# PRBonn/OverlapNet

Measured on NVIDIA H100. Metric: scan-pairs/sec (overlap+yaw) at 64x900, higher is better.
Workload: dtype f16

## Files before the change

### overlapnet_b200/csrc/network_tc.cu

```cuda
#include "common.cuh"
#include "hopper.cuh"

#include <cuda_fp16.h>
#include <stddef.h>
#include <stdlib.h>

namespace ovn {

using namespace hopper;

constexpr int WF = 360;
constexpr int CF = 128;
constexpr int S15 = 15;
constexpr int NB = 24;
constexpr int PAIR_ROWS = NB * NB;
constexpr int K4_PITCH = CF;

struct TcState {
  Buffer<__half> w1p;
  Buffer<__half> w2p;
  Buffer<__half> w3p;
  Buffer<float> b2eff;
  Buffer<__half> wres[kMaxLegLayers];
  Buffer<__half> actp[2];
// ... 463 lines not shown
              wgmma_m64n128k16_ss(acc[sub], desc_kmajor(a_base + sub * (C2_TILE / 2) + kk * 32, 16, 1024, kSwizzle128B), bd);
          }
        wgmma_commit();
        wgmma_wait<1>();
        if (di > 0) S.ring.release(gi - 1);
      }
      wgmma_wait<0>();
      if (failed) goto done;
      S.ring.release(gi - 1);
#pragma unroll
      for (int sub = 0; sub < 2; ++sub)
#pragma unroll
        for (int h = 0; h < 2; ++h) {
          const int64_t m = tile * TC_ROWS + wg * 128 + sub * 64 + wi * 16 + g + 8 * h;
          if (m >= M) continue;
#pragma unroll
          for (int j = 0; j < 16; ++j) {
            const int n = j * 8 + 2 * t;
            const float a = fmaxf(acc[sub][4 * j + 2 * h] + __ldg(bias2 + n), 0.f) - __ldg(mu_x3 + n);
            const float b = fmaxf(acc[sub][4 * j + 2 * h + 1] + __ldg(bias2 + n + 1), 0.f) - __ldg(mu_x3 + n + 1);
            *reinterpret_cast<uint32_t*>(x3 + ((size_t)j * out_pitch + m) * 8 + 2 * t) = pack_h2(a, b);
          }
        }
    }
  }
done:
  return;
}

constexpr int C3_AROWS = TC_ROWS + 2 * NB + 2;
constexpr uint32_t C3_PLANE = C3_AROWS * 16;
constexpr uint32_t C3_SLAB = 4 * 128 * 16;
constexpr int C3_GROUP = 2;
constexpr int C3_NSTAGES = 36 / C3_GROUP;
constexpr int C3_RING = 4;

struct C3Smem {
  __half A[2][16 * C3_PLANE / 2];
  __half B[C3_RING][C3_GROUP * C3_SLAB / 2];
  MbarRing<C3_RING> w3;
  MbarRing<2> x3;
};
static_assert(sizeof(C3Smem) <= 232448, "k_conv3_wgmma shared memory");
static_assert(offsetof(C3Smem, B) % 16 == 0 && C3_PLANE % 16 == 0, "bulk-copy alignment");

__global__ void __launch_bounds__(TC_THREADS, 1)
k_conv3_wgmma(const __half* __restrict__ X3, int64_t a_pitch, const __half* __restrict__ W3p, const float* __restrict__ bias,
              int64_t M, const float* __restrict__ wd, float* __restrict__ partial, int* __restrict__ err) {
  extern __shared__ __align__(128) uint8_t smem_raw[];
  C3Smem& S = *reinterpret_cast<C3Smem*>(smem_raw);
  const int tid = threadIdx.x, warp = tid >> 5, lane = tid & 31;
  const Share tiles = work_share(2 * ((M + TC_ROWS - 1) / TC_ROWS), blockIdx.x, gridDim.x);
  if (tid == 0) {
    S.w3.init(TC_WG * 4);
    S.x3.init(TC_WG * 4);
    mbar_fence_init();
  }
  __syncthreads();

  if (warp == TC_WG * 4) {
    if (lane == 0) {
      const uint32_t nt = (uint32_t)(tiles.end - tiles.begin);
      uint32_t ai = 0, gi = 0;
      for (uint32_t ti = 0; ti < nt; ++ti) {
        const int nh = (int)((tiles.begin + ti) & 1);
        for (int st = 0; st < C3_NSTAGES; ++st, ++gi) {
          while (ai < nt && ai <= ti + 1) {
            if (ai > ti) {
              if (!S.x3.try_acquire(ai, 16 * C3_PLANE)) break;
            } else {
              PIPE_WAIT(S.x3.acquire(ai, 16 * C3_PLANE), kErrConv3X3Producer);
            }
            const int64_t r0 = ((tiles.begin + ai) >> 1) * TC_ROWS;
            for (int pl = 0; pl < 16; ++pl)
              bulk_g2s(S.A[S.x3.slot(ai)] + pl * (C3_PLANE / 2), X3 + ((size_t)pl * a_pitch + r0) * 8, C3_PLANE, S.x3.bar(ai));
            ++ai;
          }
          PIPE_WAIT(S.w3.acquire(gi, C3_GROUP * C3_SLAB), kErrConv3W3Producer);
          bulk_g2s(S.B[S.w3.slot(gi)], W3p + ((size_t)nh * 36 + st * C3_GROUP) * (C3_SLAB / 2), C3_GROUP * C3_SLAB,
                   S.w3.bar(gi));
        }
      }
    }
  } else {
    const int wg = warp >> 2, wi = warp & 3, g = lane >> 2, t = lane & 3;
    const uint32_t b_base = smem_u32(S.B[0]);
    uint32_t gi = 0;
    bool failed = false;
    for (int64_t tile = tiles.begin; tile < tiles.end; ++tile) {
      const uint32_t ti = (uint32_t)(tile - tiles.begin);
      const int nh = (int)(tile & 1);
      const int64_t r0 = (tile >> 1) * TC_ROWS;
      PIPE_WAIT(S.x3.wait(ti), kErrConv3X3Consumer);
      const uint32_t a_rows = smem_u32(S.A[S.x3.slot(ti)]) + wg * 128 * 16;
      float acc[2][64];
#pragma unroll
      for (int sub = 0; sub < 2; ++sub)
#pragma unroll
        for (int e = 0; e < 64; ++e) acc[sub][e] = 0.f;
#pragma unroll 1
      for (int st = 0; st < C3_NSTAGES; ++st, ++gi) {
        const uint32_t s = S.w3.slot(gi);
        INFLIGHT_WAIT(S.w3.wait(gi), kErrConv3W3Consumer);
        wgmma_fence();
#pragma unroll
        for (int sl = 0; sl < C3_GROUP; ++sl) {
          const int slab = st * C3_GROUP + sl, tap = slab >> 2, c32 = slab & 3;
          const uint32_t a_tap = a_rows + ((tap / 3) * NB + tap % 3) * 16;
          const uint32_t slab_addr = b_base + s * (C3_GROUP * C3_SLAB) + sl * C3_SLAB;
#pragma unroll
          for (int kk = 0; kk < 2; ++kk) {
            const int c16 = c32 * 2 + kk;
            const uint64_t bd = desc_kmajor(slab_addr + kk * 4096, 2048, 128, kNoSwizzle);
#pragma unroll
            for (int sub = 0; sub < 2; ++sub)
              wgmma_m64n128k16_ss(acc[sub], desc_kmajor(a_tap + 2 * c16 * C3_PLANE + sub * 64 * 16, C3_PLANE, 128, kNoSwizzle), bd);
          }
        }
        wgmma_commit();
        wgmma_wait<1>();
        if (st > 0) S.w3.release(gi - 1);
      }
      wgmma_wait<0>();
      if (failed) goto done;
      S.w3.release(gi - 1);
      S.x3.release(ti);
#pragma unroll
      for (int sub = 0; sub < 2; ++sub)
#pragma unroll
        for (int h = 0; h < 2; ++h) {
          const int64_t r = r0 + wg * 128 + sub * 64 + wi * 16 + g + 8 * h;
          const int rem = (int)(r % PAIR_ROWS);
          const int yy = rem / NB, xx = rem - yy * NB;
          const bool valid = (r < M) && (yy < NB - 2) && (xx < NB - 2);
          const float* wrow = wd + (size_t)(valid ? (xx * (NB - 2) + yy) : 0) * 256 + nh * 128;
          float sum = 0.f;
#pragma unroll
          for (int j = 0; j < 16; ++j) {
            const int n = j * 8 + 2 * t;
            sum = fmaf(fmaxf(acc[sub][4 * j + 2 * h] + __ldg(bias + nh * 128 + n), 0.f), __ldg(wrow + n), sum);
            sum = fmaf(fmaxf(acc[sub][4 * j + 2 * h + 1] + __ldg(bias + nh * 128 + n + 1), 0.f), __ldg(wrow + n + 1), sum);
          }
          sum += __shfl_xor_sync(0xffffffffu, sum, 1);
          sum += __shfl_xor_sync(0xffffffffu, sum, 2);
          if (t == 0 && r < M) partial[r * 2 + nh] = valid ? sum : 0.f;
        }
    }
  }
done:
  return;
}

constexpr int C6_PARTS = C6_LT * C6_RT;
constexpr int C6_WG = 2;
constexpr int C6_THREADS = C6_WG * 128 + 32;
constexpr int C6_RING = 3;
constexpr int C6_GPITCH = 132;

struct C6Smem {
  __half R[C6_R_BYTES / 2];
  __half L[C6_RING][C6_L_BYTES / 2];
  float G[C6_WG][C6_LROWS * C6_GPITCH];
  MbarRing<C6_RING> left;
  MbarRing<1> right;
};
static_assert(sizeof(C6Smem) <= 232448, "k_corr_wgmma shared memory");
static_assert(offsetof(C6Smem, L) % 16 == 0, "bulk-copy alignment");

__global__ void __launch_bounds__(C6_THREADS, 1)
k_corr_wgmma(const __half* __restrict__ Lc, const int32_t* __restrict__ l_idx, const __half* __restrict__ Rc,
             int r_per_pair, int n_pairs, float* __restrict__ corr_part, int* __restrict__ err) {
  extern __shared__ __align__(128) uint8_t smem_raw[];
  C6Smem& S = *reinterpret_cast<C6Smem*>(smem_raw);
  const int tid = threadIdx.x, warp = tid >> 5, lane = tid & 31;
  const int q = blockIdx.x % C6_RT;
  const Share share = work_share((int64_t)n_pairs * C6_LT, blockIdx.x / C6_RT, gridDim.x / C6_RT);
  const int u_begin = (int)share.begin, u_end = (int)share.end;
  if (tid == 0) {
    S.left.init(4);
    S.right.init(C6_WG * 4);
    mbar_fence_init();
  }
  __syncthreads();

  if (warp == C6_WG * 4) {
    if (lane == 0) {
      uint32_t ri = 0, ui = 0;
      int key = -1;
      for (int u = u_begin; u < u_end; ++u, ++ui) {
        const int p = u / C6_LT, a = u - p * C6_LT;
        if ((r_per_pair ? p : 0) != key) {
          key = r_per_pair ? p : 0;
          PIPE_WAIT(S.right.acquire(ri, C6_R_BYTES), kErrCorrRightProducer);
          bulk_g2s(S.R, Rc + ((size_t)key * C6_RT + q) * (C6_R_BYTES / 2), C6_R_BYTES, S.right.bar(ri));
          ++ri;
        }
        PIPE_WAIT(S.left.acquire(ui, C6_L_BYTES), kErrCorrLeftProducer);
        bulk_g2s(S.L[S.left.slot(ui)], Lc + ((size_t)(l_idx ? l_idx[p] : p) * C6_LT + a) * (C6_L_BYTES / 2), C6_L_BYTES,
                 S.left.bar(ui));
      }
    }
  } else {
    const int wg = warp >> 2, wi = warp & 3, g = lane >> 2, t = lane & 3, tw = tid & 127;
    float* Gw = S.G[wg];
    const uint32_t r_base = smem_u32(S.R);
    uint32_t ri = 0, ui = 0;
    int key = -1;
    bool failed = false;
    for (int u = u_begin; u < u_end; ++u, ++ui) {
      const int p = u / C6_LT, a = u - p * C6_LT;
      if ((r_per_pair ? p : 0) != key) {
        if (key >= 0) S.right.release(ri - 1);
        key = r_per_pair ? p : 0;
        INFLIGHT_WAIT(S.right.wait(ri), kErrCorrRightConsumer);
        ++ri;
      }
      if ((int)(ui & 1) != wg) continue;
      const uint32_t s = S.left.slot(ui);
      INFLIGHT_WAIT(S.left.wait(ui), kErrCorrLeftConsumer);
      const uint32_t l_base = smem_u32(S.L[s]);
      float acc[64];
#pragma unroll
      for (int e = 0; e < 64; ++e) acc[e] = 0.f;
      wgmma_fence();
#pragma unroll
      for (int c16 = 0; c16 < 8; ++c16) {
        const uint64_t ah = desc_kmajor(l_base + c16 * 2 * C6_LROWS * 16, C6_LROWS * 16, 128, kNoSwizzle);
        const uint64_t al = desc_kmajor(l_base + C6_L_BYTES / 2 + c16 * 2 * C6_LROWS * 16, C6_LROWS * 16, 128, kNoSwizzle);
        const uint64_t bh = desc_kmajor(r_base + c16 * 2 * C6_RROWS * 16, C6_RROWS * 16, 128, kNoSwizzle);
        const uint64_t bl = desc_kmajor(r_base + C6_R_BYTES / 2 + c16 * 2 * C6_RROWS * 16, C6_RROWS * 16, 128, kNoSwizzle);
        wgmma_m64n128k16_ss(acc, ah, bh);
        wgmma_m64n128k16_ss(acc, al, bh);
        wgmma_m64n128k16_ss(acc, ah, bl);
      }
      wgmma_commit();
      wgmma_wait<0>();
      S.left.release(ui);
      named_bar_sync(1 + wg, 128);
#pragma unroll
      for (int j = 0; j < 16; ++j) {
        float* r0 = Gw + (wi * 16 + g) * C6_GPITCH + j * 8 + 2 * t;
        *reinterpret_cast<float2*>(r0) = make_float2(acc[4 * j], acc[4 * j + 1]);
        *reinterpret_cast<float2*>(r0 + 8 * C6_GPITCH) = make_float2(acc[4 * j + 2], acc[4 * j + 3]);
      }
      named_bar_sync(1 + wg, 128);
      const int i_lim = min(C6_LROWS, WF - a * C6_LROWS), j_lim = min(C6_RROWS, WF - q * C6_RROWS);
      float* out = corr_part + ((size_t)p * C6_PARTS + a * C6_RT + q) * WF;
      for (int d = tw; d < WF; d += 128) {
        const int dd = d - (C6_RROWS - 1);
        float sum = 0.f;
        if (d < C6_LROWS + C6_RROWS - 1) {
#pragma unroll 8
          for (int ii = 0; ii < C6_LROWS; ++ii) {
            const int jj = ii - dd;
            if (ii < i_lim && jj >= 0 && jj < j_lim) sum += Gw[ii * C6_GPITCH + jj];
          }
        }
        int k = (a * C6_LROWS - q * C6_RROWS + dd - WF / 2) % WF;
        if (k < 0) k += WF;
        out[k] = sum;
      }
    }
  }
done:
  return;
}

template <int EPI>
__global__ void __launch_bounds__(MMA_THREADS)
k_leg_mma(LegArgs g) {
  const int warp = threadIdx.x >> 5, lane = threadIdx.x & 31, gq = lane >> 2, t = lane & 3;
  const int64_t px0 = (int64_t)blockIdx.y * MMA_ROWS + warp * 16;
  if (px0 >= g.M) return;
  const int nz = (g.n_valid + 63) / 64;
  const int y = blockIdx.x, z = blockIdx.z % nz, slice = blockIdx.z / nz;
  const int64_t in_base = (int64_t)(y / g.runs_per_img) * g.in_img_planes + (int64_t)(y % g.runs_per_img) * g.in_run_planes;
  const int64_t pa = px0 + gq < g.M ? px0 + gq : g.M - 1, pb = px0 + gq + 8 < g.M ? px0 + gq + 8 : g.M - 1;
  const int n_slabs = g.kh * g.kw * 3;
  const size_t plane = (size_t)g.a_pitch * 8;
  const int per_tap = g.c8in / 2, n_it = g.kh * g.kw * per_tap;
  const int it0 = n_it * slice / g.n_split, it1 = n_it * (slice + 1) / g.n_split;
  float acc[8][4] = {};
#pragma unroll 1
  for (int it = it0; it < it1;) {
    const int tap = it / per_tap, dh = tap / g.kw, dw = tap - dh * g.kw;
    const int c8_end = (tap + 1) * per_tap < it1 ? g.c8in : (it1 - tap * per_tap) * 2;
    {
      const __half* Ah = g.A + (size_t)(in_base + (int64_t)dh * 2 * g.c8in) * plane + (size_t)dw * 8 + 2 * t;
      const __half* Al = Ah + (size_t)g.c8in * plane;
      const __half* Bh = g.Bp + ((size_t)(z * n_slabs + (dh * g.kw + dw) * 3) * g.c8in * 64 + gq) * 8 + 2 * t;
      const __half* Bl = Bh + (size_t)2 * g.c8in * 64 * 8;
#pragma unroll 1
      for (int c8 = (it - tap * per_tap) * 2; c8 < c8_end; c8 += 2) {
        const size_t o0 = (size_t)c8 * plane, o1 = o0 + plane;
        const uint32_t h0 = ld_h2(Ah + o0 + pa * 8), h1 = ld_h2(Ah + o0 + pb * 8), h2 = ld_h2(Ah + o1 + pa * 8), h3 = ld_h2(Ah + o1 + pb * 8);
        const uint32_t l0 = ld_h2(Al + o0 + pa * 8), l1 = ld_h2(Al + o0 + pb * 8), l2 = ld_h2(Al + o1 + pa * 8), l3 = ld_h2(Al + o1 + pb * 8);
        const size_t bo = (size_t)c8 * 64 * 8;
#pragma unroll
        for (int j = 0; j < 8; ++j) {
          const uint32_t wh0 = ld_h2(Bh + bo + j * 64), wh1 = ld_h2(Bh + bo + 64 * 8 + j * 64);
          const uint32_t wl0 = ld_h2(Bl + bo + j * 64), wl1 = ld_h2(Bl + bo + 64 * 8 + j * 64);
          mma16816(acc[j], h0, h1, h2, h3, wh0, wh1);
          mma16816(acc[j], l0, l1, l2, l3, wh0, wh1);
          mma16816(acc[j], h0, h1, h2, h3, wl0, wl1);
        }
      }
    }
    it = tap * per_tap + c8_end / 2;
  }
#pragma unroll
  for (int h = 0; h < 2; ++h) {
    const int64_t px = px0 + gq + 8 * h;
    if (px >= g.M) continue;
#pragma unroll
    for (int j = 0; j < 8; ++j) {
      const int n = z * 64 + j * 8 + 2 * t;
      if (n >= g.n_valid) continue;
      if (EPI == 5) {
        *reinterpret_cast<float2*>(g.part + (((size_t)slice * gridDim.x + y) * g.M + px) * g.n_valid + n) =
            make_float2(acc[j][2 * h], acc[j][2 * h + 1]);
        continue;
      }
      const float pre_a = acc[j][2 * h] + __ldg(g.bias + n), pre_b = acc[j][2 * h + 1] + __ldg(g.bias + n + 1);
      const float a = fmaxf(pre_a, 0.f), b = fmaxf(pre_b, 0.f);
      if (EPI == 4) {
        if (leg_act_unstorable(pre_a) || leg_act_unstorable(pre_b)) atomicCAS(g.err, 0, kErrNonFiniteOperand);
        const __half2 hi = __floats2half2_rn(a, b);
        const float2 hf = __half22float2(hi);
        const int64_t pl = (int64_t)y * g.out_run_planes + (n >> 3);
        *reinterpret_cast<__half2*>(g.out_planes + ((size_t)pl * g.out_pitch + px) * 8 + (n & 7)) = hi;
        *reinterpret_cast<uint32_t*>(g.out_planes + ((size_t)(pl + g.out_run_planes / 2) * g.out_pitch + px) * 8 + (n & 7)) =
            pack_h2(a - hf.x, b - hf.y);
      } else {
        *reinterpret_cast<float2*>(g.out_f32 + ((size_t)y * g.M + px) * g.n_valid + n) = make_float2(a, b);
      }
    }
  }
}

template <int EPI>
__global__ void __launch_bounds__(256)
k_leg_splitk_reduce(LegArgs g, int rows) {
  const int c8n = g.n_valid / 8;
  const int64_t i = (int64_t)blockIdx.x * blockDim.x + threadIdx.x;
  if (i >= (int64_t)rows * g.M * c8n) return;
  const int c8 = (int)(i % c8n);
  const int64_t px = (i / c8n) % g.M, y = i / c8n / g.M;
  const int64_t slice_stride = (int64_t)rows * g.M * g.n_valid;
  const float* src = g.part + (y * g.M + px) * g.n_valid + c8 * 8;
  float v[8] = {};
  for (int sl = 0; sl < g.n_split; ++sl) {
    const float4 a = __ldg(reinterpret_cast<const float4*>(src + sl * slice_stride));
    const float4 b = __ldg(reinterpret_cast<const float4*>(src + sl * slice_stride + 4));
    v[0] += a.x; v[1] += a.y; v[2] += a.z; v[3] += a.w; v[4] += b.x; v[5] += b.y; v[6] += b.z; v[7] += b.w;
  }
  bool bad = false;
#pragma unroll
  for (int e = 0; e < 8; ++e) {
    v[e] += __ldg(g.bias + c8 * 8 + e);
    bad |= leg_act_unstorable(v[e]);
    v[e] = fmaxf(v[e], 0.f);
  }
  if (EPI == 4) {
    if (bad) atomicCAS(g.err, 0, kErrNonFiniteOperand);
    __half hi[8], lo[8];
#pragma unroll
    for (int e = 0; e < 8; ++e) {
      hi[e] = __float2half_rn(v[e]);
      lo[e] = __float2half_rn(v[e] - __half2float(hi[e]));
    }
    const int64_t pl = y * g.out_run_planes + c8;
    *reinterpret_cast<uint4*>(g.out_planes + ((size_t)pl * g.out_pitch + px) * 8) = *reinterpret_cast<const uint4*>(hi);
    *reinterpret_cast<uint4*>(g.out_planes + ((size_t)(pl + g.out_run_planes / 2) * g.out_pitch + px) * 8) =
        *reinterpret_cast<const uint4*>(lo);
  } else {
    float* dst = g.out_f32 + (y * g.M + px) * g.n_valid + c8 * 8;
    *reinterpret_cast<float4*>(dst) = make_float4(v[0], v[1], v[2], v[3]);
    *reinterpret_cast<float4*>(dst + 4) = make_float4(v[4], v[5], v[6], v[7]);
  }
}

__global__ void __launch_bounds__(384)
k_corr_finalize(const float* __restrict__ part, float* __restrict__ corr_out, int32_t* __restrict__ yaw,
                const int* __restrict__ err) {
  __shared__ float s_corr[WF];
  const int p = blockIdx.x;
  for (int k = threadIdx.x; k < WF; k += blockDim.x) {
    float c = 0.f;
    for (int b = 0; b < C6_PARTS; ++b) c += part[((size_t)p * C6_PARTS + b) * WF + k];
    s_corr[k] = c;
    if (corr_out) corr_out[(size_t)p * WF + k] = c;
  }
  __syncthreads();
  if (threadIdx.x == 0) {
    int best = 0;
    float bv = s_corr[0];
    for (int k = 1; k < WF; ++k)
      if (s_corr[k] > bv) { bv = s_corr[k]; best = k; }
    yaw[p] = (*err != 0) ? INT32_MIN : 180 - best;
  }
}

__global__ void __launch_bounds__(1024)
k_o1_channel_mean(const __half* __restrict__ o1, int64_t M, float* __restrict__ mu) {
  __shared__ float part[16][64];
  const int o = threadIdx.x & 63, g = threadIdx.x >> 6;
  float acc = 0.f;
  for (int64_t m = g; m < M; m += 16)
    for (int di = 0; di < S15; ++di) acc += __half2float(o1[o1_chunk_offset(m, di, o >> 3) + (o & 7)]);
  part[g][o] = acc;
  __syncthreads();
  if (g == 0) {
    float t = 0.f;
    for (int k = 0; k < 16; ++k) t += part[k][o];
    mu[o] = __half2float(__float2half_rn(t / (float)(M * S15)));
  }
}

__global__ void __launch_bounds__(1024)
k_x3_channel_mean(const __half* __restrict__ x3, int64_t pitch, int64_t M, float* __restrict__ mu) {
  __shared__ float part[8][128];
  const int n = threadIdx.x & 127, g = threadIdx.x >> 7;
  float acc = 0.f;
  for (int64_t m = g; m < M; m += 8) acc += __half2float(x3[((size_t)(n >> 3) * pitch + m) * 8 + (n & 7)]);
  part[g][n] = acc;
  __syncthreads();
  if (g == 0) {
    float t = 0.f;
    for (int k = 0; k < 8; ++k) t += part[k][n];
    mu[n] = t / (float)M;
  }
}

__global__ void __launch_bounds__(128)
k_fold_bias2(const float* __restrict__ b2base, const float* __restrict__ mu_o1, const float* __restrict__ W2,
             float* __restrict__ b2eff) {
  const int n = threadIdx.x;
  float acc = b2base[n];
  for (int di = 0; di < S15; ++di)
    for (int o = 0; o < 64; ++o) acc = fmaf(mu_o1[o], W2[((size_t)di * 64 + o) * 128 + n], acc);
  b2eff[n] = acc;
}

__global__ void __launch_bounds__(256)
k_fold_bias3(const float* __restrict__ b3, const float* __restrict__ mu_x3, const float* __restrict__ W3,
             float* __restrict__ b3eff) {
  const int m = threadIdx.x;
  float acc = b3[m];
  for (int tap = 0; tap < 9; ++tap)
    for (int n = 0; n < 128; ++n)
      acc = fmaf(mu_x3[n], W3[((size_t)tap * 128 + n) * 256 + m], acc);
  b3eff[m] = acc;
}

__global__ void __launch_bounds__(256)
k_dense_finalize(const float* __restrict__ partial, const float* __restrict__ bd, int rows_per_pair,
                 float* __restrict__ overlap, const int* __restrict__ err) {
  __shared__ float red[256];
  const int p = blockIdx.x;
  const float* x = partial + (size_t)p * rows_per_pair * 2;
  float acc = 0.f;
  for (int i = threadIdx.x; i < rows_per_pair * 2; i += 256) acc += x[i];
  red[threadIdx.x] = acc;
  __syncthreads();
  for (int o = 128; o > 0; o >>= 1) {
    if (threadIdx.x < o) red[threadIdx.x] += red[threadIdx.x + o];
    __syncthreads();
  }
  if (threadIdx.x == 0) overlap[p] = (*err != 0) ? __int_as_float(0x7fc00000) : 1.0f / (1.0f + expf(-(red[0] + bd[0])));
}

constexpr size_t L1_DIRECT_SMEM = 48 * 1024;
constexpr size_t L1_SMALL_SMEM = 200 * 1024;

template <bool CIN4>
__global__ void __launch_bounds__(512, CIN4 ? 0 : 2)
k_leg_layer1_direct(const float* __restrict__ x, const float* __restrict__ w, const float* __restrict__ bias,
                    int n, int H_in, int W_in, int cin, int kh, int kw, int sh, int sw, int H_out, int W_out,
                    int relu, __half* __restrict__ out, int* __restrict__ err) {
  constexpr int CO = 16;
  extern __shared__ __align__(16) float w_s[];
  const int pairs = (W_out + 1) / 2;
  int64_t idx = (int64_t)blockIdx.x * blockDim.x + threadIdx.x;
  const bool active = idx < (int64_t)n * H_out * pairs;
  if (!active) idx = 0;
  const int xo = 2 * (int)(idx % pairs);
  const int64_t r = idx / pairs;
  const int y = (int)(r % H_out);
  const int64_t img = r / H_out;
  const bool has1 = xo + 1 < W_out;
  float acc0[CO], acc1[CO];
#pragma unroll
  for (int e = 0; e < CO; ++e) acc0[e] = acc1[e] = bias[e];
  const float* base0 = x + ((img * H_in + (int64_t)y * sh) * W_in + (int64_t)xo * sw) * cin;
  const float* base1 = has1 ? base0 + (int64_t)sw * cin : base0;
  for (int dh = 0; dh < kh; ++dh) {
    __syncthreads();
    for (int i = threadIdx.x; i < kw * cin * CO; i += blockDim.x) w_s[i] = w[(size_t)dh * kw * cin * CO + i];
    __syncthreads();
    for (int dw = 0; dw < kw; ++dw) {
      const int64_t off = ((int64_t)dh * W_in + dw) * cin;
      const float* pw = w_s + (size_t)(dw * cin) * CO;
      if (CIN4) {
        const float4 a = __ldg(reinterpret_cast<const float4*>(base0 + off));
        const float4 b = __ldg(reinterpret_cast<const float4*>(base1 + off));
        const float va[4] = {a.x, a.y, a.z, a.w}, vb[4] = {b.x, b.y, b.z, b.w};
#pragma unroll
        for (int c = 0; c < 4; ++c) {
#pragma unroll
          for (int q4 = 0; q4 < 4; ++q4) {
            const float4 wv = *reinterpret_cast<const float4*>(pw + c * CO + q4 * 4);
            acc0[q4 * 4 + 0] = fmaf(va[c], wv.x, acc0[q4 * 4 + 0]); acc1[q4 * 4 + 0] = fmaf(vb[c], wv.x, acc1[q4 * 4 + 0]);
            acc0[q4 * 4 + 1] = fmaf(va[c], wv.y, acc0[q4 * 4 + 1]); acc1[q4 * 4 + 1] = fmaf(vb[c], wv.y, acc1[q4 * 4 + 1]);
            acc0[q4 * 4 + 2] = fmaf(va[c], wv.z, acc0[q4 * 4 + 2]); acc1[q4 * 4 + 2] = fmaf(vb[c], wv.z, acc1[q4 * 4 + 2]);
            acc0[q4 * 4 + 3] = fmaf(va[c], wv.w, acc0[q4 * 4 + 3]); acc1[q4 * 4 + 3] = fmaf(vb[c], wv.w, acc1[q4 * 4 + 3]);
          }
        }
      } else {
        for (int c = 0; c < cin; ++c) {
          const float va = __ldg(base0 + off + c), vb = __ldg(base1 + off + c);
#pragma unroll
          for (int q4 = 0; q4 < 4; ++q4) {
            const float4 wv = *reinterpret_cast<const float4*>(pw + c * CO + q4 * 4);
            acc0[q4 * 4 + 0] = fmaf(va, wv.x, acc0[q4 * 4 + 0]); acc1[q4 * 4 + 0] = fmaf(vb, wv.x, acc1[q4 * 4 + 0]);
            acc0[q4 * 4 + 1] = fmaf(va, wv.y, acc0[q4 * 4 + 1]); acc1[q4 * 4 + 1] = fmaf(vb, wv.y, acc1[q4 * 4 + 1]);
            acc0[q4 * 4 + 2] = fmaf(va, wv.z, acc0[q4 * 4 + 2]); acc1[q4 * 4 + 2] = fmaf(vb, wv.z, acc1[q4 * 4 + 2]);
            acc0[q4 * 4 + 3] = fmaf(va, wv.w, acc0[q4 * 4 + 3]); acc1[q4 * 4 + 3] = fmaf(vb, wv.w, acc1[q4 * 4 + 3]);
          }
        }
      }
    }
  }
  if (!active) return;
#pragma unroll
  for (int p = 0; p < 2; ++p) {
    if (p == 1 && !has1) break;
    const float* acc = p ? acc1 : acc0;
#pragma unroll
    for (int g = 0; g < 2; ++g) {
      __half hi[8], lo[8];
      bool bad = false;
#pragma unroll
// ... 63 lines not shown
  __half hi[8], lo[8];
  bool bad = false;
#pragma unroll
  for (int e = 0; e < 8; ++e) {
    const float v = relu ? fmaxf(acc[e], 0.f) : acc[e];
    bad |= leg_act_unstorable(relu ? acc[e] : fabsf(acc[e]));
    hi[e] = __float2half_rn(v);
    lo[e] = __float2half_rn(v - __half2float(hi[e]));
  }
  if (bad) atomicCAS(err, 0, kErrNonFiniteOperand);
  const int64_t plane_hi = r * (2 * C8) + g;
  *reinterpret_cast<uint4*>(out + ((size_t)plane_hi * W_out + xo) * 8) = *reinterpret_cast<const uint4*>(hi);
  *reinterpret_cast<uint4*>(out + ((size_t)(plane_hi + C8) * W_out + xo) * 8) = *reinterpret_cast<const uint4*>(lo);
}

static int tc_supported(const ovn_handle* h) {
  return h->net_ok && h->cfg.leg_output_width == WF && h->cfg.conv1size == S15;
}

static int leg_split(const ovn_handle* h, const ConvSpec& L, int n) {
  if (n > 2) return 1;
  const int64_t tiles = (int64_t)n * L.h_out * ((L.w_out + MMA_ROWS - 1) / MMA_ROWS) * ((L.cout + 63) / 64);
  const int64_t n_it = (int64_t)L.kh * L.kw * (L.cin / 16);
  int64_t sp = (4 * h->sm_count + tiles - 1) / tiles;
  if (sp > n_it / 4) sp = n_it / 4;
  return sp < 1 ? 1 : (int)sp;
}

int tc_pack_weights(ovn_handle* h) {
  if (!tc_supported(h))
    OVN_SET_ERR(h, OVN_ERR_BAD_CONFIG, "precision f16_tc supports leg_output_width=360, conv1size=15 only");
  const ConvSpec& L1 = h->leg[0];
  const size_t l1_row_bytes = (size_t)L1.kw * L1.cin * L1.cout * sizeof(float);
  if (L1.cout != 16 || l1_row_bytes > L1_DIRECT_SMEM || l1_row_bytes * L1.kh > L1_SMALL_SMEM)
    OVN_SET_ERR(h, OVN_ERR_BAD_CONFIG, "tensor-core leg: layer %s does not fit k_leg_layer1_direct / _small", L1.name);
  h->tc.reset();
  std::unique_ptr<TcState, TcStateDelete> t(new TcState());
  const LayerWeights& w1 = h->host_w["c_conv1"];
  const LayerWeights& w2 = h->host_w["c_conv2"];
  const LayerWeights& w3 = h->host_w["c_conv3"];
  std::vector<__half> p1((size_t)K4_STEPS * 4 * 64 * 8);
  for (int cc = 0; cc < 4; ++cc)
    for (int dj = 0; dj < S15; ++dj)
      for (int k8 = 0; k8 < 4; ++k8)
        for (int o = 0; o < 64; ++o)
          for (int e = 0; e < 8; ++e) {
            const int c = cc * 32 + k8 * 8 + e;
            p1[((((size_t)(cc * S15 + dj) * 4 + k8) * 64 + o) * 8) + e] =
                __float2half(w1.kernel[((size_t)dj * CF + c) * 64 + o]);
          }
  std::vector<__half> p2((size_t)S15 * 2 * 128 * 64);
  for (int di = 0; di < S15; ++di)
    for (int n = 0; n < 128; ++n)
      for (int o = 0; o < 64; ++o) {
        const float wf = w2.kernel[((size_t)di * 64 + o) * 128 + n];
        const __half wh = __float2half(wf);
        const __half wl = __float2half(wf - __half2float(wh));
        const size_t off = (size_t)n * 64 + (((o >> 3) ^ (n & 7)) << 3) + (o & 7);
        p2[((size_t)di * 2 + 0) * 128 * 64 + off] = wh;
        p2[((size_t)di * 2 + 1) * 128 * 64 + off] = wl;
      }
  std::vector<__half> p3((size_t)2 * 36 * 4 * 128 * 8);
  for (int dy = 0; dy < 3; ++dy)
    for (int dx = 0; dx < 3; ++dx)
      for (int gq = 0; gq < 4; ++gq) {
        const int sl = (dy * 3 + dx) * 4 + gq;
        for (int nh = 0; nh < 2; ++nh)
          for (int j = 0; j < 4; ++j)
            for (int n = 0; n < 128; ++n)
              for (int e = 0; e < 8; ++e) {
                const int c = (gq * 4 + j) * 8 + e;
                p3[((((size_t)nh * 36 + sl) * 4 + j) * 128 + n) * 8 + e] =
                    __float2half(w3.kernel[(((size_t)dx * 3 + dy) * 128 + c) * 256 + nh * 128 + n]);
              }
      }
  std::vector<float> b2e(128);
  {
    const LayerWeights& wb1 = h->host_w["c_conv1"];
    for (int n = 0; n < 128; ++n) {
      double acc = w2.bias[n];
      for (int di = 0; di < S15; ++di)
        for (int o = 0; o < 64; ++o) acc += (double)wb1.bias[o] * (double)w2.kernel[((size_t)di * 64 + o) * 128 + n];
      b2e[n] = (float)acc;
    }
  }
  int rc;
  if ((rc = upload_vec(h, t->b2eff, b2e)) != OVN_OK) return rc;
  if ((rc = upload_vec(h, t->b2base, b2e)) != OVN_OK) return rc;
  if ((rc = upload_vec(h, t->b3eff, w3.bias)) != OVN_OK) return rc;
  if ((rc = t->mu_o1.ensure(h, 64 * sizeof(float))) != OVN_OK) return rc;
  OVN_CUDA(h, cudaMemset(t->mu_o1, 0, 64 * sizeof(float)));
  if ((rc = t->mu_x3.ensure(h, 128 * sizeof(float))) != OVN_OK) return rc;
  OVN_CUDA(h, cudaMemset(t->mu_x3, 0, 128 * sizeof(float)));
  if ((rc = upload_vec(h, t->w1p, p1)) != OVN_OK) return rc;
  if ((rc = upload_vec(h, t->w2p, p2)) != OVN_OK) return rc;
  if ((rc = upload_vec(h, t->w3p, p3)) != OVN_OK) return rc;
  size_t max_planes_bytes = 0;
  for (int l = 0; l < h->n_leg; ++l) {
    const ConvSpec& L = h->leg[l];
    const size_t out_bytes = (size_t)L.h_out * 2 * (L.cout / 8) * L.w_out * 16;
    if (out_bytes > max_planes_bytes) max_planes_bytes = out_bytes;
    if (l == 0) continue;
    if (L.cin % 16 != 0 || L.cout % 8 != 0 || L.sw != 1)
      OVN_SET_ERR(h, OVN_ERR_BAD_CONFIG, "tensor-core leg: layer %s shape not supported", L.name);
    const LayerWeights& w = h->host_w[L.name];
    const int c8in = L.cin / 8;
    const int nz = (L.cout + 63) / 64;
    int rc2;
    {
      const int nsl = L.kh * L.kw * 3;
      std::vector<__half> br((size_t)nz * nsl * c8in * 64 * 8, __float2half(0.f));
      for (int z = 0; z < nz; ++z)
        for (int dh = 0; dh < L.kh; ++dh)
          for (int dw = 0; dw < L.kw; ++dw)
            for (int term = 0; term < 3; ++term) {
              const int sl = (dh * L.kw + dw) * 3 + term;
              for (int c8 = 0; c8 < c8in; ++c8)
                for (int n = 0; n < 64 && z * 64 + n < L.cout; ++n)
                  for (int k = 0; k < 8; ++k) {
                    const float wf = w.kernel[(((size_t)dh * L.kw + dw) * L.cin + c8 * 8 + k) * L.cout + z * 64 + n];
                    const __half wh = __float2half(wf);
                    const __half wl = __float2half(wf - __half2float(wh));
                    br[((((size_t)z * nsl + sl) * c8in + c8) * 64 + n) * 8 + k] = (term == 2) ? wl : wh;
                  }
            }
      if ((rc2 = upload_vec(h, t->wres[l], br)) != OVN_OK) return rc2;
    }
  }
  size_t part_bytes = 0;
  for (int l = 1; l < h->n_leg; ++l)
    for (int n = 1; n <= 2 && n <= h->cfg.max_batch_scans; ++n) {
      const ConvSpec& L = h->leg[l];
      const int sp = leg_split(h, L, n);
      const size_t b = sp > 1 ? (size_t)sp * n * L.h_out * L.w_out * L.cout * sizeof(float) : 0;
      if (b > part_bytes) part_bytes = b;
    }
  if ((rc = t->leg_part.ensure(h, part_bytes)) != OVN_OK) return rc;
  for (int b = 0; b < 2; ++b) {
    const size_t bytes = max_planes_bytes * h->cfg.max_batch_scans + 32768;
    if ((rc = t->actp[b].ensure(h, bytes)) != OVN_OK) return rc;
    OVN_CUDA(h, cudaMemset(t->actp[b], 0, bytes));
  }
  const int64_t maxp = h->cfg.max_batch_pairs;
  t->rows_pad = ((maxp * PAIR_ROWS + 1024 + 255) / 256) * 256;
  if ((rc = t->l16.ensure(h, (size_t)maxp * WF * K4_PITCH * sizeof(__half))) != OVN_OK) return rc;
  if ((rc = t->r16.ensure(h, (size_t)maxp * WF * K4_PITCH * sizeof(__half))) != OVN_OK) return rc;
  OVN_CUDA(h, cudaMemset(t->l16, 0, (size_t)maxp * WF * K4_PITCH * sizeof(__half)));
  OVN_CUDA(h, cudaMemset(t->r16, 0, (size_t)maxp * WF * K4_PITCH * sizeof(__half)));
  if ((rc = t->o1.ensure(h, (size_t)120 * t->rows_pad * 8 * sizeof(__half))) != OVN_OK) return rc;
  if ((rc = t->x3.ensure(h, (size_t)16 * t->rows_pad * 8 * sizeof(__half))) != OVN_OK) return rc;
  if ((rc = t->partial.ensure(h, (size_t)t->rows_pad * 2 * sizeof(float))) != OVN_OK) return rc;
  if ((rc = t->lc.ensure(h, (size_t)maxp * C6_VOL_L_BYTES)) != OVN_OK) return rc;
  if ((rc = t->rc.ensure(h, (size_t)maxp * C6_VOL_R_BYTES)) != OVN_OK) return rc;
  if ((rc = t->corr_part.ensure(h, (size_t)maxp * C6_PARTS * WF * sizeof(float))) != OVN_OK) return rc;
  OVN_CUDA(h, cudaFuncSetAttribute(k_delta_conv1_wgmma, cudaFuncAttributeMaxDynamicSharedMemorySize, (int)sizeof(K4Smem)));
  OVN_CUDA(h, cudaFuncSetAttribute(k_conv2_wgmma, cudaFuncAttributeMaxDynamicSharedMemorySize, (int)C2_SMEM));
  OVN_CUDA(h, cudaFuncSetAttribute(k_conv3_wgmma, cudaFuncAttributeMaxDynamicSharedMemorySize, (int)sizeof(C3Smem)));
  OVN_CUDA(h, cudaFuncSetAttribute(k_corr_wgmma, cudaFuncAttributeMaxDynamicSharedMemorySize, (int)sizeof(C6Smem)));
  if ((rc = t->mu.ensure(h, CF * sizeof(float))) != OVN_OK) return rc;
  OVN_CUDA(h, cudaMemset(t->mu, 0, CF * sizeof(float)));
  OVN_CUDA(h, cudaMemset(t->o1, 0, (size_t)120 * t->rows_pad * 8 * sizeof(__half)));
  OVN_CUDA(h, cudaMemset(t->x3, 0, (size_t)16 * t->rows_pad * 8 * sizeof(__half)));
  OVN_CUDA(h, cudaFuncSetAttribute(k_leg_layer1_small<true>, cudaFuncAttributeMaxDynamicSharedMemorySize, (int)L1_SMALL_SMEM));
  OVN_CUDA(h, cudaFuncSetAttribute(k_leg_layer1_small<false>, cudaFuncAttributeMaxDynamicSharedMemorySize, (int)L1_SMALL_SMEM));
  h->tc = std::move(t);
  return OVN_OK;
}

int leg_forward_tc(ovn_handle* h, const float* d_input, int n, float* d_fv, cudaStream_t s, int stop_layer) {
  TcState* t = h->tc.get();
  if (!t) OVN_SET_ERR(h, OVN_ERR_WEIGHTS, "tensor-core weights not packed");
  prof_mark(h, PROF_LEG, s);
  {
    const ConvSpec& L = h->leg[0];
    const size_t w_bytes = (size_t)L.kw * L.cin * L.cout * sizeof(float);
    const size_t w_all = w_bytes * L.kh;
    if (n <= 2) {
      const unsigned grid = (unsigned)(((int64_t)n * L.h_out * (L.cout / 8) * L.w_out + 255) / 256);
      if (L.cin == 4)
        k_leg_layer1_small<true><<<grid, 256, w_all, s>>>(d_input, h->d_w[0], h->d_b[0], n, L.h_in, L.w_in, L.cin, L.kh, L.kw,
                                                         L.sh, L.sw, L.h_out, L.w_out, L.cout, L.relu, t->actp[0], h->d_err);
      else
        k_leg_layer1_small<false><<<grid, 256, w_all, s>>>(d_input, h->d_w[0], h->d_b[0], n, L.h_in, L.w_in, L.cin, L.kh, L.kw,
                                                          L.sh, L.sw, L.h_out, L.w_out, L.cout, L.relu, t->actp[0], h->d_err);
    } else {
      const int64_t work = (int64_t)n * L.h_out * ((L.w_out + 1) / 2);
      const unsigned grid = (unsigned)((work + 511) / 512);
      if (L.cin == 4)
        k_leg_layer1_direct<true><<<grid, 512, w_bytes, s>>>(d_input, h->d_w[0], h->d_b[0], n, L.h_in, L.w_in, L.cin, L.kh, L.kw,
                                                            L.sh, L.sw, L.h_out, L.w_out, L.relu, t->actp[0], h->d_err);
      else
        k_leg_layer1_direct<false><<<grid, 512, w_bytes, s>>>(d_input, h->d_w[0], h->d_b[0], n, L.h_in, L.w_in, L.cin, L.kh, L.kw,
                                                             L.sh, L.sw, L.h_out, L.w_out, L.relu, t->actp[0], h->d_err);
    }
    OVN_LAUNCH_CHECK(h);
  }
  int cur = 0;
  for (int l = 1; l < h->n_leg && l <= stop_layer; ++l) {
    const ConvSpec& L = h->leg[l];
    const bool last = (l == h->n_leg - 1);
    const int nz = (L.cout + 63) / 64;
    if (last && (L.cout != 128 || L.h_out != 1)) OVN_SET_ERR(h, OVN_ERR_BAD_CONFIG, "tensor-core leg: unexpected last layer");
    LegArgs la = {};
    la.A = t->actp[cur]; la.a_pitch = L.w_in; la.runs_per_img = L.h_out; la.in_img_planes = L.h_in * 2 * (L.cin / 8);
    la.in_run_planes = L.sh * 2 * (L.cin / 8); la.kh = L.kh; la.kw = L.kw; la.c8in = L.cin / 8; la.Bp = t->wres[l];
    la.bias = h->d_b[l]; la.n_valid = L.cout; la.M = L.w_out; la.out_planes = t->actp[cur ^ 1]; la.out_pitch = L.w_out;
    la.out_run_planes = 2 * (L.cout / 8); la.out_f32 = d_fv;
    la.n_split = leg_split(h, L, n); la.part = t->leg_part; la.err = h->d_err;
    const dim3 grid((unsigned)(n * L.h_out), (unsigned)((L.w_out + MMA_ROWS - 1) / MMA_ROWS), (unsigned)(nz * la.n_split));
    if (la.n_split > 1) {
      k_leg_mma<5><<<grid, MMA_THREADS, 0, s>>>(la);
      OVN_LAUNCH_CHECK(h);
      const int64_t work = (int64_t)n * L.h_out * L.w_out * (L.cout / 8);
      if (last) k_leg_splitk_reduce<3><<<(unsigned)((work + 255) / 256), 256, 0, s>>>(la, n * L.h_out);
      else k_leg_splitk_reduce<4><<<(unsigned)((work + 255) / 256), 256, 0, s>>>(la, n * L.h_out);
    } else if (last) {
      k_leg_mma<3><<<grid, MMA_THREADS, 0, s>>>(la);
    } else {
      k_leg_mma<4><<<grid, MMA_THREADS, 0, s>>>(la);
    }
    OVN_LAUNCH_CHECK(h);
    cur ^= 1;
  }
  prof_mark(h, PROF_LEG, s);
  return OVN_OK;
}

static int calibrate_all(ovn_handle* h, const float* d_vols, const int32_t* d_idx, bool keep_mu, cudaStream_t s);

int tc_bank_release(ovn_handle* h, const float* d_bank) {
  TcState* t = h->tc.get();
  if (!t || (d_bank && t->pb_key != d_bank)) return OVN_OK;
  OVN_CUDA(h, cudaDeviceSynchronize());
  t->pb_l16 = {};
  t->pb_lc = {};
  t->pb_bad = {};
  t->pb_key = nullptr;
  t->pb_rows = 0;
  return OVN_OK;
}

int tc_bank_prepare(ovn_handle* h, const float* d_bank, int64_t capacity, int64_t first, int64_t count, cudaStream_t s) {
  TcState* t = h->tc.get();
  if (!t) OVN_SET_ERR(h, OVN_ERR_WEIGHTS, "tensor-core weights not packed");
  const size_t l16_bytes = (size_t)capacity * WF * K4_PITCH * sizeof(__half);
  if (t->pb_key != d_bank || l16_bytes > t->pb_l16.bytes()) {
    int rc = OVN_OK;
    if (t->pb_key != nullptr || t->pb_l16) rc = tc_bank_release(h, nullptr);
    if (rc == OVN_OK) rc = t->pb_l16.ensure(h, l16_bytes);
    if (rc == OVN_OK) rc = t->pb_lc.ensure(h, (size_t)capacity * C6_VOL_L_BYTES);
    if (rc == OVN_OK) rc = t->pb_bad.ensure(h, (size_t)capacity * sizeof(int32_t));
    if (rc != OVN_OK) return rc;
    OVN_CUDA(h, cudaMemsetAsync(t->pb_l16, 0, l16_bytes, s));
    t->pb_key = d_bank;
    t->pb_rows = 0;
    if (first != 0) OVN_SET_ERR(h, OVN_ERR_INVALID_ARG, "ovn_bank_prepare: a new bank must be prepared from row 0");
  }
  if (first > t->pb_rows) OVN_SET_ERR(h, OVN_ERR_INVALID_ARG, "ovn_bank_prepare: rows [%lld, %lld) were never prepared",
                                      (long long)t->pb_rows, (long long)first);
  const int64_t per = (int64_t)WF * CF / 4, perL = 16 * C6_LT * C6_LROWS;
  const float* src = d_bank + (size_t)first * WF * CF;
  if (!t->mu_set) {
    int rc = calibrate_all(h, src, nullptr, false, s);
    if (rc != OVN_OK) return rc;
  }
  OVN_CUDA(h, cudaMemsetAsync(t->pb_bad + first, 0, (size_t)count * sizeof(int32_t), s));
  k_gather_rows_f16<<<(unsigned)((count * per + 255) / 256), 256, 0, s>>>(src, nullptr, (int)count, t->mu, 0,
                                                                         t->pb_l16 + (size_t)first * WF * K4_PITCH, h->d_err,
                                                                         t->pb_bad + first);
  OVN_LAUNCH_CHECK(h);
  k_pack_corr<C6_LROWS, C6_LT><<<(unsigned)((count * perL + 255) / 256), 256, 0, s>>>(src, nullptr, (int)count,
                                                                      t->pb_lc + (size_t)first * (C6_VOL_L_BYTES / 2), h->d_err,
                                                                      t->pb_bad + first);
  OVN_LAUNCH_CHECK(h);
  if (first + count > t->pb_rows) t->pb_rows = first + count;
  return OVN_OK;
}

static int calibrate_all(ovn_handle* h, const float* d_vols, const int32_t* d_idx, bool keep_mu, cudaStream_t s) {
  TcState* t = h->tc.get();
  const int base = kMaxLegLayers;
  const int64_t per = (int64_t)WF * CF / 4;
  if (!keep_mu) {
    k_channel_mean<<<1, 1024, 0, s>>>(d_vols, d_idx, 1, t->mu);
    OVN_LAUNCH_CHECK(h);
  }
  OVN_CUDA(h, cudaMemsetAsync(t->mu_o1, 0, 64 * sizeof(float), s));
  OVN_CUDA(h, cudaMemsetAsync(t->mu_x3, 0, 128 * sizeof(float), s));
  k_gather_rows_f16<<<(unsigned)((per + 255) / 256), 256, 0, s>>>(d_vols, d_idx, 1, t->mu, 0, t->l16, h->d_err, nullptr);
  OVN_LAUNCH_CHECK(h);
  k_gather_rows_f16<<<(unsigned)((per + 255) / 256), 256, 0, s>>>(d_vols, d_idx, 1, t->mu, WF / 2, t->r16, h->d_err, nullptr);
  OVN_LAUNCH_CHECK(h);
  t->last_n = 0;
  const int64_t Mc = PAIR_ROWS;
  const int g4c = NB < h->sm_count ? NB : h->sm_count;
  const int64_t tiles_c = (Mc + TC_ROWS - 1) / TC_ROWS;
  k_delta_conv1_wgmma<<<g4c, K4_THREADS, sizeof(K4Smem), s>>>(t->l16, nullptr, t->r16, 0, t->w1p, t->mu_o1, t->o1, 1, h->d_err);
  OVN_LAUNCH_CHECK(h);
  k_o1_channel_mean<<<1, 1024, 0, s>>>(t->o1, Mc, t->mu_o1);
  OVN_LAUNCH_CHECK(h);
  k_fold_bias2<<<1, 128, 0, s>>>(t->b2base, t->mu_o1, h->d_w[base + 1], t->b2eff);
  OVN_LAUNCH_CHECK(h);
  k_delta_conv1_wgmma<<<g4c, K4_THREADS, sizeof(K4Smem), s>>>(t->l16, nullptr, t->r16, 0, t->w1p, t->mu_o1, t->o1, 1, h->d_err);
  OVN_LAUNCH_CHECK(h);
  k_conv2_wgmma<<<(unsigned)tiles_c, TC_THREADS, C2_SMEM, s>>>(t->o1, t->w2p, t->b2eff, t->mu_x3, t->x3, t->rows_pad, Mc, 0,
                                                              h->d_err);
  OVN_LAUNCH_CHECK(h);
// ... 204 lines not shown
```

Baseline: 219,400.

## Reduce correlation diagonals in registers via shuffles instead of shared-memory tile

The corr epilogue no longer spills the full 64x128 fp32 accumulator tile to shared memory for a per-thread diagonal scan. Each warp now sums its accumulator fragment along anti-diagonals in registers using warp shuffles and writes a small per-warp strip, which four warps then combine. Partial outputs store only the valid diagonal span instead of the full circular width, and the finalize kernel handles the circular index remap. This cuts shared-memory traffic, removes a barrier and shrinks the partial buffer, at the cost of intricate lane-mapping logic and explicit masking of out-of-range rows and columns.

```diff
diff --git a/overlapnet_b200/csrc/network_tc.cu b/overlapnet_b200/csrc/network_tc.cu
--- a/overlapnet_b200/csrc/network_tc.cu
+++ b/overlapnet_b200/csrc/network_tc.cu
@@ -639,18 +639,56 @@
 }
 
 constexpr int C6_PARTS = C6_LT * C6_RT;
+constexpr int C6_DIAG = C6_LROWS + C6_RROWS - 1;
+constexpr int C6_STRIP = 16 + C6_RROWS;
 constexpr int C6_WG = 2;
 constexpr int C6_THREADS = C6_WG * 128 + 32;
 constexpr int C6_RING = 3;
-constexpr int C6_GPITCH = 132;
 
 struct C6Smem {
   __half R[C6_R_BYTES / 2];
   __half L[C6_RING][C6_L_BYTES / 2];
-  float G[C6_WG][C6_LROWS * C6_GPITCH];
+  float strip[C6_WG][2][4][C6_STRIP];
   MbarRing<C6_RING> left;
   MbarRing<1> right;
 };
+
+__device__ __forceinline__ void c6_strip_diagonals(const float (&acc)[64], int g, int t, float* __restrict__ out) {
+  float b[17][2];
+#pragma unroll
+  for (int e = 0; e < 2; ++e) {
+    b[0][e] = acc[2 + e];
+#pragma unroll
+    for (int jj = 0; jj < 15; ++jj) b[jj + 1][e] = acc[4 * jj + e] + acc[4 * jj + 6 + e];
+    b[16][e] = acc[60 + e];
+  }
+  float c[18][2];
+#pragma unroll
+  for (int m = 0; m < 18; ++m)
+#pragma unroll
+    for (int e = 0; e < 2; ++e) {
+      const float on = m <= 16 ? b[m][e] : 0.f, above = m >= 1 ? b[m - 1][e] : 0.f;
+      c[m][e] = 2 * t + e <= g ? on : above;
+    }
+  const int src1 = (g & 1) ? 4 * (g - 1) + ((t + 3) & 3) : 4 * (g + 1) + t;
+  float v[18];
+#pragma unroll
+  for (int m = 0; m < 18; ++m) v[m] = c[m][0] + __shfl_sync(0xffffffffu, c[m][1], src1);
+  const int hb = (g >> 1) & 1, g2 = g ^ 2;
+  const int src2 = 4 * g2 + ((t + ((g2 - g) >> 1)) & 3);
+  float w[9];
+#pragma unroll
+  for (int i = 0; i < 9; ++i)
+    w[i] = (hb ? v[2 * i + 1] : v[2 * i]) + __shfl_sync(0xffffffffu, hb ? v[2 * i] : v[2 * i + 1], src2);
+  const int qb = g >> 2, r = (g - 2 * t) & 7;
+#pragma unroll
+  for (int k = 0; k < 4; ++k) {
+    const float x = (qb ? w[2 * k + 1] : w[2 * k]) + __shfl_xor_sync(0xffffffffu, qb ? w[2 * k] : w[2 * k + 1], 18);
+    out[8 * (17 - (4 * k + 2 * qb + hb)) + r] = x;
+  }
+  const float x = w[8] + __shfl_xor_sync(0xffffffffu, w[8], 18);
+  if (!qb) out[8 * (17 - (16 + hb)) + r] = x;
+}
 static_assert(sizeof(C6Smem) <= 232448, "k_corr_wgmma shared memory");
 static_assert(offsetof(C6Smem, L) % 16 == 0, "bulk-copy alignment");
 
@@ -689,7 +727,6 @@
     }
   } else {
     const int wg = warp >> 2, wi = warp & 3, g = lane >> 2, t = lane & 3, tw = tid & 127;
-    float* Gw = S.G[wg];
     const uint32_t r_base = smem_u32(S.R);
     uint32_t ri = 0, ui = 0;
     int key = -1;
@@ -723,29 +760,28 @@
       wgmma_commit();
       wgmma_wait<0>();
       S.left.release(ui);
+      const int i_lim = min(C6_LROWS, WF - a * C6_LROWS), j_lim = min(C6_RROWS, WF - q * C6_RROWS);
+      if (i_lim < C6_LROWS || j_lim < C6_RROWS) {
+#pragma unroll
+        for (int j = 0; j < 16; ++j)
+#pragma unroll
+          for (int h = 0; h < 2; ++h)
+#pragma unroll
+            for (int e = 0; e < 2; ++e)
+              if (wi * 16 + g + 8 * h >= i_lim || j * 8 + 2 * t + e >= j_lim) acc[4 * j + 2 * h + e] = 0.f;
+      }
+      float (&strip)[4][C6_STRIP] = S.strip[wg][(ui >> 1) & 1];
+      c6_strip_diagonals(acc, g, t, strip[wi]);
       named_bar_sync(1 + wg, 128);
-#pragma unroll
-      for (int j = 0; j < 16; ++j) {
-        float* r0 = Gw + (wi * 16 + g) * C6_GPITCH + j * 8 + 2 * t;
-        *reinterpret_cast<float2*>(r0) = make_float2(acc[4 * j], acc[4 * j + 1]);
-        *reinterpret_cast<float2*>(r0 + 8 * C6_GPITCH) = make_float2(acc[4 * j + 2], acc[4 * j + 3]);
-      }
-      named_bar_sync(1 + wg, 128);
-      const int i_lim = min(C6_LROWS, WF - a * C6_LROWS), j_lim = min(C6_RROWS, WF - q * C6_RROWS);
-      float* out = corr_part + ((size_t)p * C6_PARTS + a * C6_RT + q) * WF;
-      for (int d = tw; d < WF; d += 128) {
-        const int dd = d - (C6_RROWS - 1);
-        float sum = 0.f;
-        if (d < C6_LROWS + C6_RROWS - 1) {
-#pragma unroll 8
-          for (int ii = 0; ii < C6_LROWS; ++ii) {
-            const int jj = ii - dd;
-            if (ii < i_lim && jj >= 0 && jj < j_lim) sum += Gw[ii * C6_GPITCH + jj];
-          }
-        }
-        int k = (a * C6_LROWS - q * C6_RROWS + dd - WF / 2) % WF;
-        if (k < 0) k += WF;
-        out[k] = sum;
+      float* out = corr_part + ((size_t)p * C6_PARTS + a * C6_RT + q) * C6_DIAG;
+      for (int d = tw; d < C6_DIAG; d += 128) {
+        float s[4];
+#pragma unroll
+        for (int w = 0; w < 4; ++w) {
+          const int k = d + 1 - 16 * w;
+          s[w] = k >= 0 && k < C6_STRIP ? strip[w][k] : 0.f;
+        }
+        out[d] = (s[0] + s[1]) + (s[2] + s[3]);
       }
     }
   }
@@ -874,7 +910,11 @@
   const int p = blockIdx.x;
   for (int k = threadIdx.x; k < WF; k += blockDim.x) {
     float c = 0.f;
-    for (int b = 0; b < C6_PARTS; ++b) c += part[((size_t)p * C6_PARTS + b) * WF + k];
+    for (int b = 0; b < C6_PARTS; ++b) {
+      const int a = b / C6_RT, q = b % C6_RT;
+      const int d = (k + WF + WF / 2 + C6_RROWS - 1 - a * C6_LROWS + q * C6_RROWS) % WF;
+      if (d < C6_DIAG) c += part[((size_t)p * C6_PARTS + b) * C6_DIAG + d];
+    }
     s_corr[k] = c;
     if (corr_out) corr_out[(size_t)p * WF + k] = c;
   }
@@ -1244,7 +1284,7 @@
   if ((rc = t->partial.ensure(h, (size_t)t->rows_pad * 2 * sizeof(float))) != OVN_OK) return rc;
   if ((rc = t->lc.ensure(h, (size_t)maxp * C6_VOL_L_BYTES)) != OVN_OK) return rc;
   if ((rc = t->rc.ensure(h, (size_t)maxp * C6_VOL_R_BYTES)) != OVN_OK) return rc;
-  if ((rc = t->corr_part.ensure(h, (size_t)maxp * C6_PARTS * WF * sizeof(float))) != OVN_OK) return rc;
+  if ((rc = t->corr_part.ensure(h, (size_t)maxp * C6_PARTS * C6_DIAG * sizeof(float))) != OVN_OK) return rc;
   OVN_CUDA(h, cudaFuncSetAttribute(k_delta_conv1_wgmma, cudaFuncAttributeMaxDynamicSharedMemorySize, (int)sizeof(K4Smem)));
   OVN_CUDA(h, cudaFuncSetAttribute(k_conv2_wgmma, cudaFuncAttributeMaxDynamicSharedMemorySize, (int)C2_SMEM));
   OVN_CUDA(h, cudaFuncSetAttribute(k_conv3_wgmma, cudaFuncAttributeMaxDynamicSharedMemorySize, (int)sizeof(C3Smem)));
```

New measurement: 222,800 (median of 6 runs). 1.02x the previous value.
